# TimoStoff/event_utils

Hardware: AMD Instinct MI355X
Metric: Mevents/s (voxel 5-bin 640x480) (higher is better)
Workload: dtype f32

## Files before the change

### event_utils_amd/_lib.py

```python
import ctypes
import os
from ctypes import c_char_p, c_double, c_float, c_int, c_int64, c_uint32, c_uint64, c_void_p

_HERE = os.path.dirname(os.path.abspath(__file__))
_ENV_DATA = getattr(os.environ, "_data", None)
_ENV_KEYS = {}


def getenv(name, default):
    if _ENV_DATA is None or type(_ENV_DATA) is not dict:
        return os.environ.get(name, default)
    k = _ENV_KEYS.get(name)
    if k is None:
        k = _ENV_KEYS[name] = os.fsencode(name)
    v = _ENV_DATA.get(k)
    return default if v is None else os.fsdecode(v)


LIB_PATH = os.environ.get("EVK_LIB_PATH") or os.path.join(_HERE, "csrc", "libevk.so")

EVK_IWE_ABS_POLARITY = 1
EVK_IWE_GRADIENT = 2
EVK_IWE_COMPACT = 16
EVK_POST_MIX, EVK_POST_BLUR_IWE, EVK_POST_VALUE, EVK_POST_NONE = 1, 2, 4, 8
EVK_MAX_RADIUS = 32
EVK_VOXEL_OVERWRITE, EVK_VOXEL_SPLIT_POLARITY, EVK_VOXEL_T_FROM_EVENTS = 1, 2, 4
EVK_VOXEL2_PARTITION_ONLY, EVK_VOXEL2_TILES_ONLY = 16, 32
EVK_VOXEL_DETERMINISTIC = 256
EVK_IMAGE2_NO_FIXED = 512
EVK_VOXEL2_REC4, EVK_VOXEL2_REC8, EVK_VOXEL2_NO_COUNT, EVK_VOXEL2_WG512 = 1024, 2048, 4096, 8192
EVK_VOXEL2_LIVE = 16384
EVK_COLUMNS_UNALIGNED = 65536
EVK_VOXEL2_NO_COUNT2 = 32768
EVK_STAGE_STATS, EVK_STAGE_COMPACT, EVK_STAGE_LEGACY_SCATTER = 16, 32, 64
EVK_SELECT_I16, EVK_SELECT_I32, EVK_SELECT_I64, EVK_SELECT_F32, EVK_SELECT_F64 = 0, 1, 2, 3, 4
EVK_SELECT_BOX, EVK_SELECT_NOT_HOT, EVK_SELECT_MASK, EVK_SELECT_RANDOM = 0, 1, 2, 3
EVK_PHILOX_SUBSET, EVK_PHILOX_RANDOM_XY, EVK_PHILOX_RANDOM_TP = 1, 2, 3
EVK_PHILOX_CORR_CHOICE, EVK_PHILOX_CORR_XY, EVK_PHILOX_CORR_T = 4, 5, 6
EVK_T_F32, EVK_T_F64 = 0, 1
EVK_WARP_ROTATION, EVK_WARP_XYZTHETA = 1, 2
EVK_WARP_ANGULAR_VELOCITY, EVK_WARP_PLANAR_FLOW = 3, 4
EVK_IWE_DIRECT = 32
EVK_WARP_LINVEL = 0
EVK_G_IDENT, EVK_G_EXP, EVK_G_STEP, EVK_G_EXPNEG = 0, 1, 2, 3
EVK_P_U8_PM1, EVK_P_U8, EVK_P_I8, EVK_P_F32 = 0, 1, 2, 3

P = c_void_p

# ... 121 lines not shown
    "evk_error_string": ([c_int], c_char_p),
    "evk_reduce_scratch_bytes": ([], c_int64),
    "evk_bucket_scratch_bytes": ([c_int], c_int64),
    "evk_compact_records_bytes": ([c_int64], c_int64),
    "evk_iwe_tiled_staging_bytes": ([c_int, c_int64, c_int, c_int, c_int, c_int], c_int64),
    "evk_voxel_tiled_staging_bytes": ([c_int, c_int64, c_int, c_int, c_int], c_int64),
    "evk_bucket_index_len": ([c_int, c_int64], c_int64),
    "evk_bucket_max_items": ([c_int, c_int64], c_int),
    "evk_comm_unique_id_bytes": ([], c_int),
    "evk_voxel2_max_tiles": ([], c_int),
    "evk_voxel2_index_len": ([c_int, c_int64], c_int64),
    "evk_voxel2_scratch_bytes": ([c_int, c_int64, c_int, c_int, c_int], c_int64),
    "evk_voxel2_num_tiles": ([c_int, c_int, c_int, c_int], c_int),
    "evk_voxel2_fits": ([c_int, c_int, c_int, c_int, c_int], c_int),
    "evk_num_cu": ([], c_int),
    "evk_image2_scratch_bytes": ([c_int, c_int64, c_int, c_int], c_int64),
    "evk_timestamp_images2_scratch_bytes": ([c_int, c_int64, c_int, c_int], c_int64),
    "evk_image2_indexed_scratch_bytes": ([c_int, c_int64, c_int, c_int], c_int64),
    "evk_dense_rank_scratch_bytes": ([c_int64], c_int64),
    "evk_spectral_scratch_bytes": ([c_int, c_int], c_int64),
    "evk_minmax_scratch_bytes": ([], c_int64),
    "evk_select_scratch_bytes": ([c_int64], c_int64),
    "evk_hot_pixels_scratch_bytes": ([], c_int64),
    "evk_augment_bounds_scratch_bytes": ([], c_int64),
    "evk_sort_events_scratch_bytes": ([c_int64], c_int64),
    "evk_iwe_param_band_rows": ([c_int, c_uint32, c_int, c_int], c_int),
    "evk_tsimg_band_rows": ([c_uint32, c_int, c_int], c_int),
}


# ... 38 lines not shown
```

### event_utils_amd/csrc/evk_part2.h

```cpp
#pragma once
#include <cstdio>
#include <cstring>
#include <mutex>
#include <type_traits>

#include "evk_part.h"

namespace evk {

#define V2_HDR 16
#define V2_MAX_TILES 2048
#define V2_TOTALS V2_HDR
#define V2_LIVE_PROGRESS (V2_HDR + V2_MAX_TILES)
#define V2_LIVE_STATUS (V2_LIVE_PROGRESS + 256)
#define V2_PART (V2_LIVE_STATUS + V2_MAX_TILES)
#define V2_COUNTER(T) (V2_PART + (T) + 1)
#define V2_ITEM(T) (V2_PART + 2 * (T) + 1)
#define V2_LB 10
#define EVK_VOXEL2_COUNT (1 << 20)
#define EVK_VOXEL2_COUNT2 (1 << 21)
#define V2_LOCAL_MASK ((1u << V2_LB) - 1u)
#define V2_WIDE (1u << V2_LB)
#define V2_P_MASK (~((2u << V2_LB) - 1u))
__device__ __forceinline__ void lds_barrier() { asm volatile("s_waitcnt lgkmcnt(0)\n\ts_barrier" ::: "memory"); }
// ... 30 lines not shown

struct Part2 {
    int S;
    int per_block;
    int nsc;
    int nt_pad;
    int nblk;
};

#define V2_FMT_IMGN 1
#define V2_FMT_IMGB 12
#define V2_FMT_IMGT 13
#define V2_FMT_IMGX 14
#define V2_FMT_IMGD 15
#define V2_FMT_VOX8W 9
#define V2_DELTA_SHIFT 12
#define V2_DELTA_LIMIT (1u << 20)
#define V2_CODE_SHIFT 10
__host__ __device__ constexpr int v2_fmt_lds_bytes(int rec) { return rec == V2_FMT_IMGN ? 8 : ((rec == V2_FMT_VOX8W || rec == V2_FMT_IMGT || rec == V2_FMT_IMGX || rec == V2_FMT_IMGD) ? 12 : rec); }
template <int THREADS, int EPT, int REC, typename C, bool LIVE = false>
__global__ void __launch_bounds__(THREADS, 4) k_part_sorted(const C c, int64_t n, TileGridG g, int ntiles, Part2 q, float t_first,
                                                            float t_last, float bm1, int t_from_events,
                                                            void *__restrict__ rec_, void *__restrict__ side_,
                                                            uint32_t *__restrict__ bases,
                                                            uint32_t *__restrict__ table, uint32_t *__restrict__ index,
                                                            uint32_t cap, uint32_t part, uint32_t *oob, uint32_t *host_report,
                                                            uint32_t seq, uint32_t *live_progress = nullptr,
                                                            uint32_t live_epoch = 0) {
    static_assert(!LIVE || REC == 8, "the live consumer reads 8-byte records written through");
    static_assert(REC == 8 || REC == 4 || REC == V2_FMT_IMGN || REC == V2_FMT_IMGB || REC == V2_FMT_IMGT || REC == V2_FMT_IMGX || REC == V2_FMT_IMGD || REC == V2_FMT_VOX8W, "record format");
    constexpr bool R8 = REC == 8 || REC == V2_FMT_VOX8W;
    constexpr bool IMGBT = REC == V2_FMT_IMGB || REC == V2_FMT_IMGT || REC == V2_FMT_IMGX || REC == V2_FMT_IMGD;
    constexpr bool STAGE_W = REC == V2_FMT_VOX8W || REC == V2_FMT_IMGN || IMGBT;
    constexpr bool VOX = R8 || REC == 4;
    constexpr int LB = v2_fmt_lds_bytes(REC);
    uint2 *const rec = static_cast<uint2 *>(rec_);
    float *const pw = static_cast<float *>(side_);
    uint2 *const wide2 = static_cast<uint2 *>(side_);
    constexpr int G = C::G, NG = EPT / G;
    static_assert(EPT % G == 0, "events per thread");
    constexpr int PER_MAX = (V2_MAX_TILES + THREADS - 1) / THREADS;
    extern __shared__ __attribute__((aligned(16))) unsigned char smem[];
    uint2 *sorted = reinterpret_cast<uint2 *>(smem);
    uint32_t *hist = reinterpret_cast<uint32_t *>(smem + (size_t)THREADS * EPT * LB + 16);
    uint32_t *cur = hist + ((ntiles + 4) & ~3);
    uint32_t *tot = cur + ((ntiles + 4) & ~3);
// ... 43 lines not shown
    auto load_xy = [&](int sc) {
#pragma unroll
        for (int k = 0; k < NG; ++k) c.template load_xy<true>(row_base(sc, k), valid_in(sc, k) > 0 ? (uint32_t)tl_ : 0u, xyr + C::XYW * k);
    };
    auto load_tp = [&](int sc) {
#pragma unroll
        for (int k = 0; k < NG; ++k) c.template load_tp<true>(row_base(sc, k), valid_in(sc, k) > 0 ? (uint32_t)tl_ : 0u, tpr + C::TPW * k);
        if constexpr (REC == 4) tb = c.t1((int64_t)sc * q.S);
    };
    auto fence = [&]() {
        asm volatile("" ::: "memory");
        __builtin_amdgcn_sched_barrier(0);
    };
    for (int i = tid; i < ntiles; i += THREADS) hist[i] = 0, tot[i] = 0;
    if (tid < 8) tmp[64 + tid] = 0;
    if (sc0 < sc_end) load_xy(sc0);
    EVK_WAIT_VM0();
    lds_barrier();
    uint32_t kept_prev = 0;
    int64_t lo_prev = 0;
    int sc_prev = 0;
    auto store_run = [&](const uint4 *src, uint4 *dst, const int n16) {
        if constexpr (REC != 4) {
            typedef uint32_t u4v __attribute__((ext_vector_type(4)));
            const __amdgpu_buffer_rsrc_t rs = __builtin_amdgcn_make_buffer_rsrc(
                (void *)dst, 0, (int)__builtin_amdgcn_readfirstlane(n16 * 16), 0x00020000);
            for (int i = tid; i < n16; i += THREADS) {
                const uint4 v = src[i];
                __builtin_amdgcn_raw_buffer_store_b128(u4v{v.x, v.y, v.z, v.w}, rs, i * 16, 0,  16);
            }
        } else {
// ... 5 lines not shown
        if constexpr (R8 || IMGBT)
            store_run(src, reinterpret_cast<uint4 *>(rec + lo_prev), (int)((kept_prev + 1) >> 1));
        else
            store_run(src, reinterpret_cast<uint4 *>(reinterpret_cast<uint32_t *>(rec_) + lo_prev), (int)((kept_prev + 3) >> 2));
        if constexpr (LIVE)
            store_run(reinterpret_cast<const uint4 *>(trow_l), reinterpret_cast<uint4 *>(table + (int64_t)sc_prev * q.nt_pad), q.nt_pad >> 2);
        if constexpr (STAGE_W) {
            if (tmp[65])
                store_run(reinterpret_cast<const uint4 *>(sortedp),
                          reinterpret_cast<uint4 *>(static_cast<uint32_t *>(side_) + lo_prev), (int)((kept_prev + 3) >> 2));
        }
    };
    for (int sc = sc0; sc < sc_end; ++sc) {
        asm volatile("" : "+v"(tl_));
        const int64_t lo = (int64_t)sc * q.S;
        if (sc > sc0) write_out();
#pragma unroll
        for (int k = 0; k < NG; ++k) {
            const int nv = valid_in(sc, k);
#pragma unroll
            for (int e = 0; e < G; ++e) {
                uint32_t cell = 0;
                int key;
                if constexpr (IMGBT) key = c.key_rel(xyr + C::XYW * k, e, g, xr[G * k + e], yr[G * k + e]);
                else key = c.key_of(xyr + C::XYW * k, e, g, cell);
                kl[G * k + e] = ((key >= 0) & (e < nv)) ? (((uint32_t)key << V2_LB) | cell) : 0xFFFFFFFFu;
                if constexpr (VOX) dropped += ((key < 0) & (e < nv)) ? 1u : 0u;
                else dropped += ((key == -1) & (e < nv)) ? 1u : 0u;
                if constexpr (IMGBT) rare |= ((key == -3) & (e < nv)) ? (1u << (G * k + e)) : 0u;
                asm volatile("" : "+v"(dropped));
                __builtin_amdgcn_sched_barrier(0);
// ... 56 lines not shown
        if constexpr (VOX) {
#pragma unroll
            for (int s2 = 0; s2 < EPT; ++s2) {
                tv[s2] = time_norm(c.t_of(tpr + C::TPW * (s2 / G), s2 % G), tnorm);
                __builtin_amdgcn_sched_barrier(0);
            }
        }
        EVK_WAIT_VM0();
        fence();
        if constexpr (EARLY) {
            if (sc == sc_end - 1 && tid == 0) {
                EVK_HANDOVER_RELEASE();
                early_prev = __hip_atomic_fetch_add(index + 8, 1u, __ATOMIC_RELAXED, __HIP_MEMORY_SCOPE_AGENT);
            }
        }
        if (sc + 1 < sc_end) load_xy(sc + 1);
        fence();
        uint32_t pos_[EPT];
#pragma unroll
        for (int s2 = 0; s2 < EPT; ++s2) {
            pos_[s2] = 0;
            if (kl[s2] != 0xFFFFFFFFu) pos_[s2] = atomicAdd(&cur[kl[s2] >> V2_LB], 1u);
        }
        auto slot_of = [&](int s2) -> uint32_t { return pos_[s2]; };
        if constexpr (REC == V2_FMT_VOX8W) {
            bool any_wide = false;
#pragma unroll
            for (int s2 = 0; s2 < EPT; ++s2) {
                if (kl[s2] != 0xFFFFFFFFu) {
                    const uint32_t pos = slot_of(s2);
                    const uint32_t pbits = __float_as_uint(c.p_of(tpr + C::TPW * (s2 / G), s2 % G));
                    const bool wide = ((pbits & ~V2_P_MASK) != 0u) | ((pbits & 0x7F800000u) == 0x7F800000u);
                    nwide += ((((pbits & 0x7FFFFFFFu) == 0x3F800000u) | (pbits == 0u)) ? 0u : 0x10000u) + (wide ? 1u : 0u);
                    sorted[pos] = make_uint2(__float_as_uint(tv[s2]), (wide ? V2_WIDE : (pbits & V2_P_MASK)) | (kl[s2] & V2_LOCAL_MASK));
                    sortedp[pos] = pbits;
                    any_wide |= wide;
                }
            }
            if (any_wide) tmp[65] = 1u;
        } else if constexpr (REC == 8) {
            uint32_t wide_mask = 0;
#pragma unroll
            for (int s2 = 0; s2 < EPT; ++s2) {
                if (kl[s2] != 0xFFFFFFFFu) {
                    const uint32_t pos = slot_of(s2);
                    const uint32_t pbits = __float_as_uint(c.p_of(tpr + C::TPW * (s2 / G), s2 % G));
                    const bool wide = ((pbits & ~V2_P_MASK) != 0u) | ((pbits & 0x7F800000u) == 0x7F800000u);
                    nwide += (((pbits & 0x7FFFFFFFu) == 0x3F800000u) | (pbits == 0u)) ? 0u : 0x10000u;
                    sorted[pos] = make_uint2(__float_as_uint(tv[s2]), (wide ? V2_WIDE : (pbits & V2_P_MASK)) | (kl[s2] & V2_LOCAL_MASK));
                    if (wide) wide_mask |= 1u << s2, kl[s2] = pos;
                }
            }
            if (__any(wide_mask != 0u)) {
#pragma unroll
                for (int s2 = 0; s2 < EPT; ++s2)
// ... 99 lines not shown
                        ++nwide;
                    }
                }
                if (live) sorted4[slot_of(s2)] = word;
            }
        }
        lds_barrier();
        if constexpr (EARLY) {
            if (sc == sc_end - 1 && tid == 0 && early_prev == gridDim.x - 1) early_publish();
        }
        if constexpr (LIVE) {
            if (sc > sc0 && tid == 0)
                __hip_atomic_store(live_progress + blockIdx.x, (live_epoch << 8) | (uint32_t)(sc - sc0), __ATOMIC_RELAXED,
                                   __HIP_MEMORY_SCOPE_AGENT);
        }
        EVK_WAIT_VM0();
        kept_prev = kept, lo_prev = lo, sc_prev = sc;
    }
    uint32_t *gidx = index;
    if constexpr (EARLY) {
        if (sc0 >= sc_end && tid == 0) {
            early_prev = __hip_atomic_fetch_add(index + 8, 1u, __ATOMIC_RELAXED, __HIP_MEMORY_SCOPE_AGENT);
            if (early_prev == gridDim.x - 1) early_publish();
        }
    } else {
        if (dropped && oob) atomicAdd(oob, dropped);
    }
    for (int i = tid; i < ntiles; i += THREADS)
        if (tot[i]) __hip_atomic_fetch_add(gidx + V2_TOTALS + i, tot[i], __ATOMIC_RELAXED, __HIP_MEMORY_SCOPE_AGENT);
    {
        uint32_t nw = nwide & 0xFFFFu, nu = nwide >> 16;
// ... 61 lines not shown
    for (int k = 0; k < PER_MAX; ++k) {
        const int i = i0 + k;
        if (k < per && i < i1) {
            const uint32_t parts = tt[k] > cap ? (tt[k] + part - 1) / part : 1u;
            part_start[i] = prun;
            counters[i] = 0;
            for (uint32_t jj = 0; jj < parts; ++jj) item_tile[prun + jj] = (uint32_t)i;
            prun += parts;
        }
    }
    if (tid == 0) {
        part_start[ntiles] = total_parts;
        __hip_atomic_store(gidx + 2, 0u, __ATOMIC_RELAXED, __HIP_MEMORY_SCOPE_AGENT);
        __hip_atomic_store(gidx + 7, now5 != prev6 ? 1u : 0u, __ATOMIC_RELAXED, __HIP_MEMORY_SCOPE_AGENT);
        __hip_atomic_store(gidx + 6, now5, __ATOMIC_RELAXED, __HIP_MEMORY_SCOPE_AGENT);
        if constexpr (!VOX) {
            __hip_atomic_store(gidx + 1, now3 != prev0 ? 1u : 0u, __ATOMIC_RELAXED, __HIP_MEMORY_SCOPE_AGENT);
            __hip_atomic_store(gidx + 0, now3, __ATOMIC_RELAXED, __HIP_MEMORY_SCOPE_AGENT);
        }
        if (!EARLY && host_report) {
            const uint32_t cnt = cnt_oob;
            __hip_atomic_store(reinterpret_cast<unsigned long long *>(host_report),
                               (unsigned long long)seq | ((unsigned long long)cnt << 32), __ATOMIC_RELAXED, __HIP_MEMORY_SCOPE_SYSTEM);
        }
    }
}

struct V2Config {
    int threads, ept;
};
#define V2_GEOMETRIES(X) X(1024, 8) X(1024, 12)
static const V2Config &v2_config(bool share = false, int ntiles = 0) {
    static const V2Config small{1024, 8}, large{1024, 12};
    return (share || ntiles <= 680) ? small : large;
}
#define V2_MIN_SUBCHUNK 8192
#define V2_LDS_LIMIT (160 * 1024 - 512)
static size_t v2_part_lds(int threads, int ept, int rec, int ntiles, bool live = false) {
    return (size_t)threads * ept * v2_fmt_lds_bytes(rec) + 16 + 3 * (size_t)((ntiles + 4) & ~3) * 4 + 72 * 4 + 16 +
           (live ? (size_t)((ntiles + 15) & ~15) * 4 + 16 : 0);
}

static Part2 v2_geometry(int64_t n, int ntiles, bool share = false) {
    const V2Config &c = v2_config(share, ntiles);
    const int64_t smax = (int64_t)c.threads * c.ept;
    int64_t nblk = (n + V2_MIN_SUBCHUNK - 1) / V2_MIN_SUBCHUNK;
    const int64_t maxblk = (int64_t)EVK_NUM_CU * (1024 / c.threads);
    if (nblk > maxblk) nblk = maxblk;
    if (nblk < 1) nblk = 1;
    int64_t per_block = (n + nblk * smax - 1) / (nblk * smax);
    if (per_block < 1) per_block = 1;
    int64_t S = (n + nblk * per_block - 1) / (nblk * per_block);
    S = (S + 3) & ~(int64_t)3;
    if (S < 4) S = 4;
    Part2 q;
    q.S = (int)S, q.per_block = (int)per_block, q.nblk = (int)nblk;
    q.nsc = (int)((n + S - 1) / S);
    if (q.nsc < 1) q.nsc = 1;
    q.nt_pad = (ntiles + 15) & ~15;
    return q;
}
static inline int64_t al256(int64_t b) { return (b + 255) & ~(int64_t)255; }
// ... 7 lines not shown
}
static int64_t v2_part(int64_t n, int ntiles) {
    const int64_t c = (int64_t)(V2_SPLIT_PART * (double)v2_mean(n, ntiles));
    return c > 8192 ? c : 8192;
}
static int v2_max_items(int64_t n, int ntiles) { return ntiles + (int)(n / v2_part(n, ntiles)) + 1; }

static int v2_rec_bytes(int64_t n, int flags) {
    if (flags & EVK_VOXEL2_REC4) return 4;
    if (flags & EVK_VOXEL2_REC8) return 8;
    return n * 16 > ((int64_t)256 << 20) ? 4 : 8;
}
struct V2Layout {
    int64_t table, bases, rec, pw, staging, total;
};
static V2Layout v2_layout(int ntiles, int64_t n, int planes, int tw, int th, bool share = false) {
    const Part2 q = v2_geometry(n, ntiles, share);
    const int64_t slots = (int64_t)q.nsc * q.S;
    V2Layout L;
    L.table = 0;
    L.bases = al256((int64_t)q.nsc * q.nt_pad * 4);
    L.rec = L.bases + al256((int64_t)q.nsc * 4);
    L.pw = L.rec + al256(slots * 8);
    L.staging = L.pw + al256(slots * 8);
    L.total = L.staging + al256((int64_t)v2_max_items(n, ntiles) * v2_staging_stride((int64_t)planes * tw * th) * 8);
    return L;
}

template <int THREADS, int EPT, int REC, typename C, bool LIVE = false>
static void launch_part(const C &c, int64_t n, const TileGridG &g, int ntiles, const Part2 &q, float t_first, float t_last,
                        float bm1, int t_from_events, void *rec, void *pw, uint32_t *bases, uint32_t *table, uint32_t *index,
                        uint32_t *oob, uint32_t *host_report, uint32_t seq, hipStream_t s, uint32_t *live_progress = nullptr,
// ... 16 lines not shown
```

### event_utils_amd/csrc/evk_voxel2.hip

```cpp
#include <atomic>

#include <hip/hip_ext.h>

#include "evk_part2.h"
#include "evk_voxel_live.h"

namespace evk {

__host__ __device__ constexpr int v2_max_chunks(int wg) { return wg == 768 ? 6 : 7; }
__host__ __device__ constexpr int v2_chunk_cap(int wg) { return 64 * v2_max_chunks(wg); }
#define V2_FIXED_ONE 4294967296.0
struct Band {
    int tile_lo, tile_hi, y_lo, rows;
};
template <int WG, int U, bool SPLIT, bool FIXED, int REC>
__global__ void __launch_bounds__(WG, REC == 4 ? 4 : 6) k_voxel_tiles2(const void *__restrict__ rec_, const void *__restrict__ side_,
                                                     const uint32_t *__restrict__ bases,
                                                     const uint32_t *__restrict__ table, uint32_t *__restrict__ index,
                                                     TileGridG g, Part2 q, int B, int flags, float *__restrict__ vox,
                                                     float *__restrict__ staging, Band band, uint32_t *live_status = nullptr,
                                                     uint32_t live_epoch = 0) {
    constexpr int NW = WG / 64, E = REC == 4 ? 3 : 1;
    typedef typename std::conditional<REC == 8, uint4, uint2>::type Pair;
    const float *const pw = static_cast<const float *>(side_);
// ... 569 lines not shown
}

}

using namespace evk;

extern "C" int64_t evk_voxel2_index_len(int ntiles, int64_t n) {
    if (ntiles <= 0 || ntiles > V2_MAX_TILES || n < 0) return 0;
    return (int64_t)V2_ITEM(ntiles) + v2_max_items(n, ntiles);
}

extern "C" int64_t evk_voxel2_scratch_bytes(int ntiles, int64_t n, int planes, int tile_w, int tile_h) {
    if (ntiles <= 0 || n < 0 || planes <= 0 || tile_w <= 0 || tile_h <= 0) return 0;
    const int64_t a = v2_layout(ntiles, n, planes, tile_w, tile_h, false).total;
    const int64_t b = v2_layout(ntiles, n, planes, tile_w, tile_h, true).total;
    return a > b ? a : b;
}

extern "C" int evk_voxel2_num_tiles(int h, int wd, int tile_w, int tile_h) {
    TileGridG g;
    if (make_grid_g(g, h, wd, tile_w, tile_h) != EVK_OK) return 0;
    if (v2_part_lds(1024, 12, 8, g.tiles_x * g.tiles_y) > (size_t)V2_LDS_LIMIT) return 0;
    return g.tiles_x * g.tiles_y;
}

static size_t v2_tiles_lds(const TileGridG &g, int planes) {
    return (size_t)planes * sizeof(acc_t) * g.pitch * g.th + 12 * 8 * (v2_chunk_cap(512) + 1) + 64;
}
#define V2_TILES_LDS_LIMIT (150 * 1024)

extern "C" int evk_voxel2_fits(int h, int wd, int tile_w, int tile_h, int planes) {
    TileGridG g;
    if (planes <= 0 || make_grid_g(g, h, wd, tile_w, tile_h) != EVK_OK) return 0;
    const int ntiles = evk_voxel2_num_tiles(h, wd, tile_w, tile_h);
    if (ntiles <= 0 || ntiles > evk_voxel2_max_tiles()) return 0;
    return v2_tiles_lds(g, planes) <= (size_t)V2_TILES_LDS_LIMIT ? 1 : 0;
}
extern "C" int evk_num_cu(void) { return EVK_NUM_CU; }

extern "C" int evk_voxel2_max_tiles(void) {
    const int64_t budget = (int64_t)V2_LDS_LIMIT - (int64_t)1024 * 12 * 8 - 1024;
    const int64_t t = budget / 12;
    return (int)(t < V2_MAX_TILES ? (t > 0 ? t : 0) : V2_MAX_TILES);
}



template <int WG, int U, bool SPLIT, bool FIXED, int REC>
static void launch_tiles(int items, size_t lds_dyn, hipStream_t s, const void *rec, const void *pw, const uint32_t *bases,
                         const uint32_t *table, uint32_t *index, const TileGridG &g, const Part2 &q, int B, int kf, float *vox,
                         float *staging, const Band &band, uint32_t *live_status = nullptr, uint32_t live_epoch = 0) {
    static std::once_flag once[64];
    int dev = 0;
    (void)hipGetDevice(&dev);
    std::call_once(once[dev & 63], [] {
        (void)hipFuncSetAttribute((const void *)k_voxel_tiles2<WG, U, SPLIT, FIXED, REC>, hipFuncAttributeMaxDynamicSharedMemorySize,
                                  160 * 1024 - (REC == 4 ? 12 : 8) * (WG / 64) * (v2_chunk_cap(WG) + 1) - 256);
    });
    k_voxel_tiles2<WG, U, SPLIT, FIXED, REC><<<items, WG, lds_dyn, s>>>(rec, pw, bases, table, index, g, q, B, kf, vox, staging, band,
// ... 33 lines not shown
static bool v2_live_fits(const TileGridG &g, int ntiles, const Part2 &q, int64_t n, int B, int recb, const V2Config &cfg) {
    const size_t acc = (size_t)2 * B * g.pitch * g.th * 8;
    return recb == 8 && cfg.threads == 1024 && cfg.ept == 8 && ntiles <= 2 * EVK_NUM_CU && q.nblk <= V2L_PROGRESS_WORDS &&
           q.per_block >= 2 && q.per_block <= 255 && n < ((int64_t)1 << 28) && (int64_t)q.nsc * q.S * 8 < ((int64_t)1 << 32) &&
           acc + V2L_STATIC_LDS <= (size_t)V2L_LDS_REQUEST &&
           v2_part_lds(1024, 8, 8, ntiles, true) + 256 + V2L_LDS_REQUEST <= (size_t)160 * 1024;
}

template <typename C>
static int voxel2(const C &c, int64_t n, int h, int wd, int tile_w, int tile_h, float t_first, float t_last, int B,
                  int flags, float *vox, uint32_t *index, void *scratch, int64_t scratch_bytes, uint32_t *oob,
                  uint32_t *host_report, uint32_t seq, void *stream, const Band &band = Band{0, 0, 0, 0}) {
    TileGridG g;
    const int known = EVK_VOXEL_OVERWRITE | EVK_VOXEL_SPLIT_POLARITY | EVK_VOXEL_T_FROM_EVENTS | EVK_VOXEL2_PARTITION_ONLY |
                      EVK_VOXEL2_TILES_ONLY | EVK_VOXEL2_NO_XCD_ORDER | EVK_VOXEL2_SHARE_CU | EVK_VOXEL_DETERMINISTIC |
                      EVK_VOXEL2_REC4 | EVK_VOXEL2_REC8 | EVK_VOXEL2_NO_COUNT | EVK_VOXEL2_WG512 | EVK_VOXEL2_LIVE | EVK_VOXEL2_NO_COUNT2;
    if (make_grid_g(g, h, wd, tile_w, tile_h) != EVK_OK || B <= 0 || !vox || !index || !scratch || n <= 0 ||
        n > (int64_t)4000000000LL || (flags & ~known))
        return EVK_EINVAL;
    if (host_report && ((uintptr_t)host_report & 7u)) return EVK_EALIGN;
    const int ntiles = g.tiles_x * g.tiles_y;
    if (ntiles > evk_voxel2_max_tiles() || !evk_voxel2_num_tiles(h, wd, tile_w, tile_h)) return EVK_EINVAL;
    const int planes = (flags & EVK_VOXEL_SPLIT_POLARITY) ? 2 * B : B;
    const size_t lds_acc = (size_t)planes * sizeof(acc_t) * g.pitch * g.th;
    if (v2_tiles_lds(g, planes) > (size_t)V2_TILES_LDS_LIMIT) return EVK_EINVAL;
    const bool share = flags & EVK_VOXEL2_SHARE_CU;
    const V2Layout L = v2_layout(ntiles, n, planes, tile_w, tile_h, share);
    if (scratch_bytes < L.total) return EVK_ESCRATCH;
    if (!aligned16(scratch)) return EVK_EALIGN;
    const Part2 q = v2_geometry(n, ntiles, share);
    char *sb = (char *)scratch;
    uint32_t *table = (uint32_t *)(sb + L.table), *bases = (uint32_t *)(sb + L.bases);
    void *rec = sb + L.rec, *pw = sb + L.pw;
    float *staging = (float *)(sb + L.staging);
    hipStream_t s = (hipStream_t)stream;
    const V2Config &cfg = v2_config(share, ntiles);
    const float bm1 = (float)(B - 1);
    const int tfe = (flags & EVK_VOXEL_T_FROM_EVENTS) ? 1 : 0;
    const int recb = v2_rec_bytes(n, flags);
    bool live = false;
    hipStream_t s2 = nullptr;
    hipEvent_t live_done = nullptr;
    uint32_t epoch = 0;
    if constexpr (std::is_same<C, SrcF32>::value) {
        if ((flags & EVK_VOXEL2_LIVE) && band.tile_hi == 0 &&
            !(flags & (EVK_VOXEL2_PARTITION_ONLY | EVK_VOXEL2_TILES_ONLY | EVK_VOXEL_SPLIT_POLARITY | EVK_VOXEL2_SHARE_CU |
                       EVK_VOXEL2_NO_COUNT)) &&
            v2_live_fits(g, ntiles, q, n, B, recb, cfg)) {
            hipStreamCaptureStatus cap = hipStreamCaptureStatusNone;
            if (hipStreamIsCapturing(s, &cap) == hipSuccess && cap == hipStreamCaptureStatusNone && (s2 = v2_live_stream()) != nullptr)
                live = true, epoch = v2_live_epoch();
            else
                (void)hipGetLastError();
        }
    }
    uint32_t *const live_progress = index + V2_LIVE_PROGRESS, *const live_status = index + V2_LIVE_STATUS;
    if (live) {
        if constexpr (std::is_same<C, SrcF32>::value) {
            launch_part<1024, 8, 8, C, true>(c, n, g, ntiles, q, t_first, t_last, bm1, tfe, rec, pw, bases, table, index, oob,
                                             host_report, seq, s, live_progress, epoch);
            LiveArgs la{live_progress, live_status, epoch, (uint32_t)v2_cap(n, ntiles), 400u};
            k_voxel_live<2><<<(ntiles + 1) / 2, V2L_WG, V2L_LDS_REQUEST - V2L_STATIC_LDS, s2>>>(
                rec, (uint32_t)((int64_t)q.nsc * q.S * 8), table, g, q, B, flags & EVK_VOXEL_OVERWRITE, vox, la);
            live_done = v2_live_event();
            if (!live_done || hipEventRecord(live_done, s2) != hipSuccess) live_done = nullptr, (void)hipGetLastError();
        }
    } else if (!(flags & EVK_VOXEL2_TILES_ONLY)) {
        if (recb == 8 && cfg.threads == 1024 && cfg.ept == 8 && !share) {
            launch_part<1024, 8, V2_FMT_VOX8W>(c, n, g, ntiles, q, t_first, t_last, bm1, tfe, rec, pw, bases, table, index, oob,
                                               host_report, seq, s);
        } else {
#define X(T, E)                                                                                                              \
    if (cfg.threads == T && cfg.ept == E) {                                                                                  \
        if (recb == 4)                                                                                                       \
            launch_part<T, E, 4>(c, n, g, ntiles, q, t_first, t_last, bm1, tfe, rec, pw, bases, table, index, oob, host_report, seq, s); \
        else                                                                                                                 \
            launch_part<T, E, 8>(c, n, g, ntiles, q, t_first, t_last, bm1, tfe, rec, pw, bases, table, index, oob, host_report, seq, s); \
    }
            V2_GEOMETRIES(X)
#undef X
        }
    }
    if (!(flags & EVK_VOXEL2_PARTITION_ONLY)) {
        const int items = v2_max_items(n, ntiles);
        int kf = flags & (EVK_VOXEL_OVERWRITE | EVK_VOXEL_SPLIT_POLARITY | EVK_VOXEL2_NO_XCD_ORDER);
        const bool sp = flags & EVK_VOXEL_SPLIT_POLARITY, fx = flags & EVK_VOXEL_DETERMINISTIC;
        const size_t lds_count = ((size_t)(B + 1) * sizeof(acc_t) + (size_t)B * 4) * g.pitch * g.th;
        auto two_fit = [](size_t acc_bytes, int wg, int rec) {
            return 2 * (acc_bytes + (size_t)(rec == 4 ? 12 : 8) * (wg / 64) * (v2_chunk_cap(wg) + 1) + 256) <= (size_t)160 * 1024;
        };
        const bool may_count = !sp && !(flags & EVK_VOXEL2_NO_COUNT) && n < ((int64_t)1 << 31);
#define V2_TILES(W, R)                                                                                                     \
// ... 87 lines not shown
```

### event_utils_amd/tiled.py

```python
import os

from . import _device as D
from . import _lib


def default_impl():
    return _lib.getenv("EVK_IMPL", "auto")


FORCE = {"rec": None, "count": True, "tiles_wg": 0, "xcd_order": True, "share_cu": None, "iwe_records": "auto",
         "iwe_fixed": True, "image_fixed": True, "live": None, "count2": True, "legacy_scatter": False, "native_bfgs": True}


TILED_MIN_EVENTS = 1
TILED_MIN_EVENTS_NATIVE = 1
TILED_MIN_EVENTS_NEG_POS = 1
TILED_MIN_EVENTS_IWE = 150_000
TILED_MIN_EVENTS_IWE_REUSED = 1
LIVE_MIN_EVENTS = 6_000_000
_WIN_MAX = {1: 64, 3: 48}
_persist = {}


class _BoundedCache(dict):

    def __setitem__(self, k, v):
# ... 250 lines not shown
        _staging_bytes[key] = sizes
    index = _zbuf(ver + "_index", sizes[0], dev)
    scratch = _buf(ver + "_scratch", sizes[1], dev)
    flags = _lib.EVK_VOXEL_SPLIT_POLARITY if split_polarity else 0
    if share_cu():
        flags |= 128
    if not FORCE["xcd_order"]:
        flags |= 64
    flags |= {None: 0, 4: _lib.EVK_VOXEL2_REC4, 8: _lib.EVK_VOXEL2_REC8}[FORCE["rec"]]
    if not FORCE["count"]:
        flags |= _lib.EVK_VOXEL2_NO_COUNT
    if not FORCE.get("count2", True):
        flags |= _lib.EVK_VOXEL2_NO_COUNT2
    if FORCE["tiles_wg"] == 512:
        flags |= _lib.EVK_VOXEL2_WG512
    live = FORCE["live"]
    if live is None:
        live = n >= LIVE_MIN_EVENTS and _lib.getenv("EVK_VOXEL_LIVE", "0") == "1"
    if live and not split_polarity and not (flags & 128):
        flags |= _lib.EVK_VOXEL2_LIVE
    if voxel_deterministic():
        flags |= _lib.EVK_VOXEL_DETERMINISTIC
    return index, scratch, sizes[1], flags


def voxel2_band_rows(H, W, B, nbands):
    shape = voxel2_shape(H, W, B)
    if shape is None:
        return None
    th = shape[1]
# ... 643 lines not shown
```

### include/evk.h

```cpp
#ifndef EVK_H
#define EVK_H

#include <stdint.h>

#ifdef __cplusplus
extern "C" {
#endif

#define EVK_VERSION 100

#define EVK_OK 0
#define EVK_EINVAL (-1)
#define EVK_ESCRATCH (-2)
#define EVK_EALIGN (-3)
#define EVK_ECOMM (-4)

#define EVK_IWE_ABS_POLARITY 1u
#define EVK_IWE_GRADIENT 2u

int evk_version(void);
const char *evk_error_string(int code);


int evk_image_nearest_i32(const int32_t *x, const int32_t *y, const int32_t *w, int64_t n, int canvas_h,
// ... 185 lines not shown
int evk_voxel_tiled_f32(const float *records, uint32_t *bucket_index, int64_t n, int h, int wd, int tw_log2, int th_log2,
                        float t_first, float t_last, int B, int flags, float *vox, void *staging,
                        int64_t staging_bytes, void *stream);

#define EVK_VOXEL_T_FROM_EVENTS 4
#define EVK_VOXEL_DETERMINISTIC 256
#define EVK_VOXEL2_PARTITION_ONLY 16
#define EVK_VOXEL2_TILES_ONLY 32
#define EVK_VOXEL2_SHARE_CU 128
#define EVK_VOXEL2_NO_XCD_ORDER 64
#define EVK_VOXEL2_REC4 1024
#define EVK_VOXEL2_REC8 2048
#define EVK_VOXEL2_NO_COUNT 4096
#define EVK_VOXEL2_WG512 8192
#define EVK_VOXEL2_NO_COUNT2 32768
#define EVK_VOXEL2_LIVE 16384
#define EVK_COLUMNS_UNALIGNED 65536
int evk_voxel2_max_tiles(void);
int64_t evk_voxel2_index_len(int ntiles, int64_t n);
int evk_voxel2_num_tiles(int h, int wd, int tile_w, int tile_h);
int evk_voxel2_fits(int h, int wd, int tile_w, int tile_h, int planes);
int evk_num_cu(void);
int64_t evk_voxel2_scratch_bytes(int ntiles, int64_t n, int planes, int tile_w, int tile_h);
int evk_voxel2_f32(const float *x, const float *y, const float *t, const float *p, int64_t n, int h, int wd,
                   int tile_w, int tile_h, float t_first, float t_last, int B, int flags, float *vox,
                   uint32_t *index, void *scratch, int64_t scratch_bytes, uint32_t *oob, uint32_t *host_report,
                   uint32_t seq, void *stream);
int evk_voxel2_band_f32(int64_t n, int h, int wd, int tile_w, int tile_h, int B, int flags, int tile_row_lo, int tile_row_hi,
                        float *band, uint32_t *index, void *scratch, int64_t scratch_bytes, void *stream);
int evk_normalise_time_f32(const float *t, int64_t n, float t_first, float t_last, int B, float *out, void *stream);
// ... 169 lines not shown
```

Baseline: 141,300.

## Add co-resident two-workgroup-per-CU partition variant with adaptive host selection

Adds a VOX8C record format for the partition kernel. It sets launch bounds for two 1024-thread workgroups per CU, doubles the maximum block count, and drops the software prefetch of the next subchunk's coordinates, loading them synchronously each iteration. Occupancy is meant to hide latency in place of the explicit prefetch. The host keeps per-index state in mapped pinned memory and falls back to the one-workgroup path when the kernel reports a non-unit condition. The cost is more scratch, per-call host bookkeeping under a mutex, and a dependency on state carried between calls.

```diff
diff --git a/event_utils_amd/_lib.py b/event_utils_amd/_lib.py
--- a/event_utils_amd/_lib.py
+++ b/event_utils_amd/_lib.py
@@ -32,6 +32,7 @@
 EVK_VOXEL2_LIVE = 16384
 EVK_COLUMNS_UNALIGNED = 65536
 EVK_VOXEL2_NO_COUNT2 = 32768
+EVK_VOXEL2_ONE_WG = 131072
 EVK_STAGE_STATS, EVK_STAGE_COMPACT, EVK_STAGE_LEGACY_SCATTER = 16, 32, 64
 EVK_SELECT_I16, EVK_SELECT_I32, EVK_SELECT_I64, EVK_SELECT_F32, EVK_SELECT_F64 = 0, 1, 2, 3, 4
 EVK_SELECT_BOX, EVK_SELECT_NOT_HOT, EVK_SELECT_MASK, EVK_SELECT_RANDOM = 0, 1, 2, 3
@@ -183,6 +184,9 @@
     "evk_voxel2_num_tiles": ([c_int, c_int, c_int, c_int], c_int),
     "evk_voxel2_fits": ([c_int, c_int, c_int, c_int, c_int], c_int),
     "evk_num_cu": ([], c_int),
+    "evk_voxel2_geometry": ([c_int64, c_int, c_int, P], c_int),
+    "evk_voxel2_last_coresident": ([P], c_int),
+    "evk_voxel2_forget_index": ([P], c_int),
     "evk_image2_scratch_bytes": ([c_int, c_int64, c_int, c_int], c_int64),
     "evk_timestamp_images2_scratch_bytes": ([c_int, c_int64, c_int, c_int], c_int64),
     "evk_image2_indexed_scratch_bytes": ([c_int, c_int64, c_int, c_int], c_int64),
diff --git a/event_utils_amd/csrc/evk_part2.h b/event_utils_amd/csrc/evk_part2.h
--- a/event_utils_amd/csrc/evk_part2.h
+++ b/event_utils_amd/csrc/evk_part2.h
@@ -68,22 +68,26 @@
 #define V2_FMT_IMGX 14
 #define V2_FMT_IMGD 15
 #define V2_FMT_VOX8W 9
+#define V2_FMT_VOX8C 10
 #define V2_DELTA_SHIFT 12
 #define V2_DELTA_LIMIT (1u << 20)
 #define V2_CODE_SHIFT 10
-__host__ __device__ constexpr int v2_fmt_lds_bytes(int rec) { return rec == V2_FMT_IMGN ? 8 : ((rec == V2_FMT_VOX8W || rec == V2_FMT_IMGT || rec == V2_FMT_IMGX || rec == V2_FMT_IMGD) ? 12 : rec); }
+__host__ __device__ constexpr int v2_fmt_lds_bytes(int rec) { return (rec == V2_FMT_IMGN || rec == V2_FMT_VOX8C) ? 8 : ((rec == V2_FMT_VOX8W || rec == V2_FMT_IMGT || rec == V2_FMT_IMGX || rec == V2_FMT_IMGD) ? 12 : rec); }
 template <int THREADS, int EPT, int REC, typename C, bool LIVE = false>
-__global__ void __launch_bounds__(THREADS, 4) k_part_sorted(const C c, int64_t n, TileGridG g, int ntiles, Part2 q, float t_first,
+__global__ void __launch_bounds__(THREADS, REC == V2_FMT_VOX8C ? 8 : 4) k_part_sorted(const C c, int64_t n, TileGridG g, int ntiles, Part2 q, float t_first,
                                                             float t_last, float bm1, int t_from_events,
                                                             void *__restrict__ rec_, void *__restrict__ side_,
                                                             uint32_t *__restrict__ bases,
                                                             uint32_t *__restrict__ table, uint32_t *__restrict__ index,
                                                             uint32_t cap, uint32_t part, uint32_t *oob, uint32_t *host_report,
-                                                            uint32_t seq, uint32_t *live_progress = nullptr,
-                                                            uint32_t live_epoch = 0) {
+                                                            uint32_t seq, uint32_t *aux = nullptr,
+                                                            uint32_t aux_seq = 0) {
+    uint32_t *const live_progress = aux;
+    const uint32_t live_epoch = aux_seq;
     static_assert(!LIVE || REC == 8, "the live consumer reads 8-byte records written through");
-    static_assert(REC == 8 || REC == 4 || REC == V2_FMT_IMGN || REC == V2_FMT_IMGB || REC == V2_FMT_IMGT || REC == V2_FMT_IMGX || REC == V2_FMT_IMGD || REC == V2_FMT_VOX8W, "record format");
-    constexpr bool R8 = REC == 8 || REC == V2_FMT_VOX8W;
+    constexpr bool CO = REC == V2_FMT_VOX8C;
+    static_assert(REC == 8 || REC == 4 || CO || REC == V2_FMT_IMGN || REC == V2_FMT_IMGB || REC == V2_FMT_IMGT || REC == V2_FMT_IMGX || REC == V2_FMT_IMGD || REC == V2_FMT_VOX8W, "record format");
+    constexpr bool R8 = REC == 8 || REC == V2_FMT_VOX8W || CO;
     constexpr bool IMGBT = REC == V2_FMT_IMGB || REC == V2_FMT_IMGT || REC == V2_FMT_IMGX || REC == V2_FMT_IMGD;
     constexpr bool STAGE_W = REC == V2_FMT_VOX8W || REC == V2_FMT_IMGN || IMGBT;
     constexpr bool VOX = R8 || REC == 4;
@@ -157,7 +161,9 @@
     };
     for (int i = tid; i < ntiles; i += THREADS) hist[i] = 0, tot[i] = 0;
     if (tid < 8) tmp[64 + tid] = 0;
-    if (sc0 < sc_end) load_xy(sc0);
+    if constexpr (!CO) {
+        if (sc0 < sc_end) load_xy(sc0);
+    }
     EVK_WAIT_VM0();
     lds_barrier();
     uint32_t kept_prev = 0;
@@ -193,7 +199,15 @@
     for (int sc = sc0; sc < sc_end; ++sc) {
         asm volatile("" : "+v"(tl_));
         const int64_t lo = (int64_t)sc * q.S;
+        if constexpr (CO) {
+            load_xy(sc);
+            fence();
+        }
         if (sc > sc0) write_out();
+        if constexpr (CO) {
+            EVK_WAIT_VM0();
+            fence();
+        }
 #pragma unroll
         for (int k = 0; k < NG; ++k) {
             const int nv = valid_in(sc, k);
@@ -280,7 +294,9 @@
                 early_prev = __hip_atomic_fetch_add(index + 8, 1u, __ATOMIC_RELAXED, __HIP_MEMORY_SCOPE_AGENT);
             }
         }
-        if (sc + 1 < sc_end) load_xy(sc + 1);
+        if constexpr (!CO) {
+            if (sc + 1 < sc_end) load_xy(sc + 1);
+        }
         fence();
         uint32_t pos_[EPT];
 #pragma unroll
@@ -304,7 +320,7 @@
                 }
             }
             if (any_wide) tmp[65] = 1u;
-        } else if constexpr (REC == 8) {
+        } else if constexpr (REC == 8 || CO) {
             uint32_t wide_mask = 0;
 #pragma unroll
             for (int s2 = 0; s2 < EPT; ++s2) {
@@ -434,7 +450,8 @@
                 __hip_atomic_store(live_progress + blockIdx.x, (live_epoch << 8) | (uint32_t)(sc - sc0), __ATOMIC_RELAXED,
                                    __HIP_MEMORY_SCOPE_AGENT);
         }
-        EVK_WAIT_VM0();
+        if constexpr (!CO)
+            EVK_WAIT_VM0();
         kept_prev = kept, lo_prev = lo, sc_prev = sc;
     }
     uint32_t *gidx = index;
@@ -526,6 +543,12 @@
         __hip_atomic_store(gidx + 2, 0u, __ATOMIC_RELAXED, __HIP_MEMORY_SCOPE_AGENT);
         __hip_atomic_store(gidx + 7, now5 != prev6 ? 1u : 0u, __ATOMIC_RELAXED, __HIP_MEMORY_SCOPE_AGENT);
         __hip_atomic_store(gidx + 6, now5, __ATOMIC_RELAXED, __HIP_MEMORY_SCOPE_AGENT);
+        if constexpr (VOX && !LIVE) {
+            if (aux)
+                __hip_atomic_store(reinterpret_cast<unsigned long long *>(aux),
+                                   (unsigned long long)aux_seq | ((unsigned long long)(now5 != prev6 ? 1u : 0u) << 32),
+                                   __ATOMIC_RELAXED, __HIP_MEMORY_SCOPE_SYSTEM);
+        }
         if constexpr (!VOX) {
             __hip_atomic_store(gidx + 1, now3 != prev0 ? 1u : 0u, __ATOMIC_RELAXED, __HIP_MEMORY_SCOPE_AGENT);
             __hip_atomic_store(gidx + 0, now3, __ATOMIC_RELAXED, __HIP_MEMORY_SCOPE_AGENT);
@@ -553,11 +576,20 @@
            (live ? (size_t)((ntiles + 15) & ~15) * 4 + 16 : 0);
 }
 
-static Part2 v2_geometry(int64_t n, int ntiles, bool share = false) {
-    const V2Config &c = v2_config(share, ntiles);
+static int v2_max_tiles() {
+    const int64_t budget = (int64_t)V2_LDS_LIMIT - (int64_t)1024 * 12 * 8 - 1024;
+    const int64_t t = budget / 12;
+    return (int)(t < V2_MAX_TILES ? (t > 0 ? t : 0) : V2_MAX_TILES);
+}
+static bool v2_co_fits(int ntiles) {
+    return ntiles > 0 && ntiles <= 680 && 2 * v2_part_lds(1024, 8, V2_FMT_VOX8C, ntiles) <= (size_t)V2_LDS_LIMIT;
+}
+
+static Part2 v2_geometry(int64_t n, int ntiles, bool share = false, bool co = false) {
+    const V2Config &c = v2_config(share || co, ntiles);
     const int64_t smax = (int64_t)c.threads * c.ept;
     int64_t nblk = (n + V2_MIN_SUBCHUNK - 1) / V2_MIN_SUBCHUNK;
-    const int64_t maxblk = (int64_t)EVK_NUM_CU * (1024 / c.threads);
+    const int64_t maxblk = (int64_t)EVK_NUM_CU * (1024 / c.threads) * (co ? 2 : 1);
     if (nblk > maxblk) nblk = maxblk;
     if (nblk < 1) nblk = 1;
     int64_t per_block = (n + nblk * smax - 1) / (nblk * smax);
@@ -595,8 +627,8 @@
 struct V2Layout {
     int64_t table, bases, rec, pw, staging, total;
 };
-static V2Layout v2_layout(int ntiles, int64_t n, int planes, int tw, int th, bool share = false) {
-    const Part2 q = v2_geometry(n, ntiles, share);
+static V2Layout v2_layout(int ntiles, int64_t n, int planes, int tw, int th, bool share = false, bool co = false) {
+    const Part2 q = v2_geometry(n, ntiles, share, co);
     const int64_t slots = (int64_t)q.nsc * q.S;
     V2Layout L;
     L.table = 0;
diff --git a/event_utils_amd/csrc/evk_voxel2.hip b/event_utils_amd/csrc/evk_voxel2.hip
--- a/event_utils_amd/csrc/evk_voxel2.hip
+++ b/event_utils_amd/csrc/evk_voxel2.hip
@@ -607,7 +607,75 @@
     if (ntiles <= 0 || n < 0 || planes <= 0 || tile_w <= 0 || tile_h <= 0) return 0;
     const int64_t a = v2_layout(ntiles, n, planes, tile_w, tile_h, false).total;
     const int64_t b = v2_layout(ntiles, n, planes, tile_w, tile_h, true).total;
-    return a > b ? a : b;
+    const int64_t c = v2_co_fits(ntiles) ? v2_layout(ntiles, n, planes, tile_w, tile_h, false, true).total : 0;
+    return a > b ? (a > c ? a : c) : (b > c ? b : c);
+}
+
+extern "C" int evk_voxel2_geometry(int64_t n, int ntiles, int flags, int *out) {
+    if (ntiles <= 0 || ntiles > V2_MAX_TILES || n <= 0 || !out) return -1;
+    const bool share = flags & EVK_VOXEL2_SHARE_CU;
+    const bool co = !share && !(flags & (EVK_VOXEL2_ONE_WG | EVK_VOXEL2_LIVE)) && v2_rec_bytes(n, flags) == 8 && v2_co_fits(ntiles);
+    const Part2 q = v2_geometry(n, ntiles, share, co);
+    out[0] = q.S, out[1] = q.per_block, out[2] = q.nsc, out[3] = q.nblk;
+    return co ? 1 : 0;
+}
+
+#define V2_STATE_SLOTS 64
+struct V2IndexState {
+    const void *index = nullptr;
+    uint32_t issued = 0;
+    bool nonunit = false, co = false;
+};
+static std::mutex v2_state_mu;
+static V2IndexState v2_state[V2_STATE_SLOTS];
+static int v2_state_next = 0;
+static unsigned long long *v2_state_words = nullptr;
+static int v2_state_find(const void *index) {
+    for (int i = 0; i < V2_STATE_SLOTS; ++i)
+        if (v2_state[i].index == index) return i;
+    return -1;
+}
+extern "C" int evk_voxel2_last_coresident(const uint32_t *index) {
+    std::lock_guard<std::mutex> lk(v2_state_mu);
+    const int i = v2_state_find(index);
+    return i < 0 ? -1 : (v2_state[i].co ? 1 : 0);
+}
+extern "C" int evk_voxel2_forget_index(const uint32_t *index) {
+    std::lock_guard<std::mutex> lk(v2_state_mu);
+    const int i = v2_state_find(index);
+    if (i >= 0) v2_state[i].index = nullptr, v2_state[i].nonunit = false, v2_state[i].co = false;
+    return EVK_OK;
+}
+static bool v2_choose_co(const void *index, bool eligible, bool want_report, hipStream_t s, uint32_t **word, uint32_t *seq) {
+    std::lock_guard<std::mutex> lk(v2_state_mu);
+    if (!v2_state_words && want_report) {
+        hipStreamCaptureStatus cap = hipStreamCaptureStatusNone;
+        void *mem = nullptr;
+        if (hipStreamIsCapturing(s, &cap) == hipSuccess && cap == hipStreamCaptureStatusNone &&
+            hipHostMalloc(&mem, V2_STATE_SLOTS * sizeof(unsigned long long), hipHostMallocPortable | hipHostMallocMapped) == hipSuccess) {
+            memset(mem, 0, V2_STATE_SLOTS * sizeof(unsigned long long));
+            v2_state_words = static_cast<unsigned long long *>(mem);
+        } else {
+            (void)hipGetLastError();
+        }
+    }
+    int i = v2_state_find(index);
+    if (i < 0) {
+        i = v2_state_next, v2_state_next = (v2_state_next + 1) % V2_STATE_SLOTS;
+        v2_state[i].index = index, v2_state[i].nonunit = false;
+    }
+    V2IndexState &st = v2_state[i];
+    if (v2_state_words && st.issued) {
+        const unsigned long long w = __atomic_load_n(v2_state_words + i, __ATOMIC_RELAXED);
+        if ((uint32_t)w == st.issued) st.nonunit = (w >> 32) != 0;
+    }
+    st.co = eligible && !st.nonunit;
+    *word = nullptr, *seq = 0;
+    if (v2_state_words && want_report) {
+        if (++st.issued == 0u) st.issued = 1u;
+        *word = reinterpret_cast<uint32_t *>(v2_state_words + i), *seq = st.issued;
+    }
+    return st.co;
 }
 
 extern "C" int evk_voxel2_num_tiles(int h, int wd, int tile_w, int tile_h) {
@@ -631,11 +699,7 @@
 }
 extern "C" int evk_num_cu(void) { return EVK_NUM_CU; }
 
-extern "C" int evk_voxel2_max_tiles(void) {
-    const int64_t budget = (int64_t)V2_LDS_LIMIT - (int64_t)1024 * 12 * 8 - 1024;
-    const int64_t t = budget / 12;
-    return (int)(t < V2_MAX_TILES ? (t > 0 ? t : 0) : V2_MAX_TILES);
-}
+extern "C" int evk_voxel2_max_tiles(void) { return v2_max_tiles(); }
 
 
 
@@ -699,7 +763,8 @@
     TileGridG g;
     const int known = EVK_VOXEL_OVERWRITE | EVK_VOXEL_SPLIT_POLARITY | EVK_VOXEL_T_FROM_EVENTS | EVK_VOXEL2_PARTITION_ONLY |
                       EVK_VOXEL2_TILES_ONLY | EVK_VOXEL2_NO_XCD_ORDER | EVK_VOXEL2_SHARE_CU | EVK_VOXEL_DETERMINISTIC |
-                      EVK_VOXEL2_REC4 | EVK_VOXEL2_REC8 | EVK_VOXEL2_NO_COUNT | EVK_VOXEL2_WG512 | EVK_VOXEL2_LIVE | EVK_VOXEL2_NO_COUNT2;
+                      EVK_VOXEL2_REC4 | EVK_VOXEL2_REC8 | EVK_VOXEL2_NO_COUNT | EVK_VOXEL2_WG512 | EVK_VOXEL2_LIVE | EVK_VOXEL2_NO_COUNT2 |
+                      EVK_VOXEL2_ONE_WG;
     if (make_grid_g(g, h, wd, tile_w, tile_h) != EVK_OK || B <= 0 || !vox || !index || !scratch || n <= 0 ||
         n > (int64_t)4000000000LL || (flags & ~known))
         return EVK_EINVAL;
@@ -710,14 +775,9 @@
     const size_t lds_acc = (size_t)planes * sizeof(acc_t) * g.pitch * g.th;
     if (v2_tiles_lds(g, planes) > (size_t)V2_TILES_LDS_LIMIT) return EVK_EINVAL;
     const bool share = flags & EVK_VOXEL2_SHARE_CU;
-    const V2Layout L = v2_layout(ntiles, n, planes, tile_w, tile_h, share);
-    if (scratch_bytes < L.total) return EVK_ESCRATCH;
+    if (scratch_bytes < evk_voxel2_scratch_bytes(ntiles, n, planes, tile_w, tile_h)) return EVK_ESCRATCH;
     if (!aligned16(scratch)) return EVK_EALIGN;
-    const Part2 q = v2_geometry(n, ntiles, share);
-    char *sb = (char *)scratch;
-    uint32_t *table = (uint32_t *)(sb + L.table), *bases = (uint32_t *)(sb + L.bases);
-    void *rec = sb + L.rec, *pw = sb + L.pw;
-    float *staging = (float *)(sb + L.staging);
+    Part2 q = v2_geometry(n, ntiles, share);
     hipStream_t s = (hipStream_t)stream;
     const V2Config &cfg = v2_config(share, ntiles);
     const float bm1 = (float)(B - 1);
@@ -739,6 +799,18 @@
                 (void)hipGetLastError();
         }
     }
+    const bool co_ok = recb == 8 && !share && !live && !(flags & EVK_VOXEL2_ONE_WG) && cfg.threads == 1024 && cfg.ept == 8 &&
+                       v2_co_fits(ntiles);
+    uint32_t *unit_word = nullptr, unit_seq = 0;
+    bool co;
+    if (flags & EVK_VOXEL2_TILES_ONLY) co = co_ok && evk_voxel2_last_coresident(index) == 1;
+    else co = v2_choose_co(index, co_ok, !live, s, &unit_word, &unit_seq);
+    if (co) q = v2_geometry(n, ntiles, share, true);
+    const V2Layout L = v2_layout(ntiles, n, planes, tile_w, tile_h, share, co);
+    char *sb = (char *)scratch;
+    uint32_t *table = (uint32_t *)(sb + L.table), *bases = (uint32_t *)(sb + L.bases);
+    void *rec = sb + L.rec, *pw = sb + L.pw;
+    float *staging = (float *)(sb + L.staging);
     uint32_t *const live_progress = index + V2_LIVE_PROGRESS, *const live_status = index + V2_LIVE_STATUS;
     if (live) {
         if constexpr (std::is_same<C, SrcF32>::value) {
@@ -751,16 +823,19 @@
             if (!live_done || hipEventRecord(live_done, s2) != hipSuccess) live_done = nullptr, (void)hipGetLastError();
         }
     } else if (!(flags & EVK_VOXEL2_TILES_ONLY)) {
-        if (recb == 8 && cfg.threads == 1024 && cfg.ept == 8 && !share) {
+        if (co) {
+            launch_part<1024, 8, V2_FMT_VOX8C>(c, n, g, ntiles, q, t_first, t_last, bm1, tfe, rec, pw, bases, table, index, oob,
+                                               host_report, seq, s, unit_word, unit_seq);
+        } else if (recb == 8 && cfg.threads == 1024 && cfg.ept == 8 && !share) {
             launch_part<1024, 8, V2_FMT_VOX8W>(c, n, g, ntiles, q, t_first, t_last, bm1, tfe, rec, pw, bases, table, index, oob,
-                                               host_report, seq, s);
+                                               host_report, seq, s, unit_word, unit_seq);
         } else {
 #define X(T, E)                                                                                                              \
     if (cfg.threads == T && cfg.ept == E) {                                                                                  \
         if (recb == 4)                                                                                                       \
-            launch_part<T, E, 4>(c, n, g, ntiles, q, t_first, t_last, bm1, tfe, rec, pw, bases, table, index, oob, host_report, seq, s); \
+            launch_part<T, E, 4>(c, n, g, ntiles, q, t_first, t_last, bm1, tfe, rec, pw, bases, table, index, oob, host_report, seq, s, unit_word, unit_seq); \
         else                                                                                                                 \
-            launch_part<T, E, 8>(c, n, g, ntiles, q, t_first, t_last, bm1, tfe, rec, pw, bases, table, index, oob, host_report, seq, s); \
+            launch_part<T, E, 8>(c, n, g, ntiles, q, t_first, t_last, bm1, tfe, rec, pw, bases, table, index, oob, host_report, seq, s, unit_word, unit_seq); \
     }
             V2_GEOMETRIES(X)
 #undef X
diff --git a/event_utils_amd/tiled.py b/event_utils_amd/tiled.py
--- a/event_utils_amd/tiled.py
+++ b/event_utils_amd/tiled.py
@@ -9,7 +9,8 @@
 
 
 FORCE = {"rec": None, "count": True, "tiles_wg": 0, "xcd_order": True, "share_cu": None, "iwe_records": "auto",
-         "iwe_fixed": True, "image_fixed": True, "live": None, "count2": True, "legacy_scatter": False, "native_bfgs": True}
+         "iwe_fixed": True, "image_fixed": True, "live": None, "count2": True, "legacy_scatter": False, "native_bfgs": True,
+         "part_one_wg": False}
 
 
 TILED_MIN_EVENTS = 1
@@ -290,6 +291,8 @@
         flags |= _lib.EVK_VOXEL2_NO_COUNT2
     if FORCE["tiles_wg"] == 512:
         flags |= _lib.EVK_VOXEL2_WG512
+    if FORCE.get("part_one_wg"):
+        flags |= _lib.EVK_VOXEL2_ONE_WG
     live = FORCE["live"]
     if live is None:
         live = n >= LIVE_MIN_EVENTS and _lib.getenv("EVK_VOXEL_LIVE", "0") == "1"
diff --git a/include/evk.h b/include/evk.h
--- a/include/evk.h
+++ b/include/evk.h
@@ -223,6 +223,10 @@
 #define EVK_VOXEL2_NO_COUNT 4096
 #define EVK_VOXEL2_WG512 8192
 #define EVK_VOXEL2_NO_COUNT2 32768
+#define EVK_VOXEL2_ONE_WG 131072
+int evk_voxel2_geometry(int64_t n, int ntiles, int flags, int *out4);
+int evk_voxel2_last_coresident(const uint32_t *index);
+int evk_voxel2_forget_index(const uint32_t *index);
 #define EVK_VOXEL2_LIVE 16384
 #define EVK_COLUMNS_UNALIGNED 65536
 int evk_voxel2_max_tiles(void);
```

Measured after the change: 135,100. 4.4% lower.
